# cyberlife-coder/velesdb

Measured on AMD Instinct MI355X. Metric: qps_at_recall10_1Mx768_k10, higher is better.
Workload: dtype f32; 1 GPU; 1000000x768 f32 cosine, k=10, exact distance sweep + fused GPU top-k (BASELINE configs[1]); 1024 queries/step, 1024 queries per corpus pass (sweep_topk_gemm_bf16_pp<dot, WIDE> over normalised bf16 images of rows and queries (cosine; ping-po; rows=1000000, dim=768, k=10, parallelism=replicas x1 (query stream split, no collective)

## Files before the change

velesdb_amd/csrc/g16_protocol.inc:

```
#ifndef VDB_PP_STAMP_AT
#define VDB_PP_STAMP_AT(SLOT) do { } while (0)
#define VDB_G16_OWN_STAMP_STUB 1
#endif
#ifndef VDB_PP_STAMP_COUNT
#define VDB_PP_STAMP_COUNT(SLOT) do { } while (0)
#define VDB_PP_STAMP_ADD(SLOT, N) do { } while (0)
#endif
    VDB_PP_STAMP_AT(16);
    if (hm[0] | hm[1] | hm[2] | hm[3]) VDB_PP_STAMP_COUNT(19);
    VDB_PP_STAMP_ADD(22, __popcll(hm[0]) + __popcll(hm[1]) + __popcll(hm[2]) + __popcll(hm[3]));
    for (;;) {
      ++epoch;
      VDB_PP_STAMP_COUNT(23);
      bool pend = false;
      {
        const uint32_t ln1 = lane_now();
        uint32_t fill = qcnt;
        uint32_t hsz = 64u;
        bool stop = false;
#define VDB_G16_SCAN(T) \
        while (hm[T] && !stop) { \
          if (hsz == 1u && fill + 32u > (uint32_t)QCAP) {  \
            stop = true; \
            break; \
          } \
          const uint32_t hrank = __builtin_amdgcn_mbcnt_hi((uint32_t)(hm[T] >> 32), __builtin_amdgcn_mbcnt_lo((uint32_t)hm[T], 0u)); \
          const bool mine = (((hm[T] >> ln1) & 1ull) != 0) & (hrank < hsz); \
          const uint64_t msk = __ballot(mine); \
          uint32_t nf = fill; \
          const uint32_t hi0 = ((uint32_t)(wr * 128) + 4u * (ln1 >> 4)) | (((uint32_t)(wq * 64 + (T) * 16) + (ln1 & 15u)) << 8); \
_Pragma("unroll") \
          for (int g8 = 0; g8 < 4; g8++) { \
            if (!__ballot(mine & (((gmv[T] >> g8) & 1u) != 0u))) continue;  \
_Pragma("unroll") \
            for (int j8 = 0; j8 < 8; j8++) { \
              float x; \
              VDB_G16_ACC_ELEM(x, acc[(8 * g8 + j8) >> 2][T][(8 * g8 + j8) & 3]);  \
               \
              const float xt = METRIC == kJaccard ? __builtin_fmaf(-cpv[T], vns[wr * 128 + 4 * (int)(ln1 >> 4) + ((8 * g8 + j8) >> 2) * 16 + ((8 * g8 + j8) & 3)], x) : x; \
              const bool pass = mine & !(xt < thrv[T]); \
              const uint64_t pm = __ballot(pass); \
              if (pm) { \
                if (pass) { \
                  const uint32_t slot = min(nf + __builtin_amdgcn_mbcnt_hi((uint32_t)(pm >> 32), __builtin_amdgcn_mbcnt_lo((uint32_t)pm, 0u)), (uint32_t)QCAP); \
                  uint32_t hi = hi0; \
                  asm volatile("" : "+v"(hi));  \
                  wq_keys[slot] = ((uint64_t)(hi + (uint32_t)(((8 * g8 + j8) >> 2) * 16 + ((8 * g8 + j8) & 3))) << 32) | (uint64_t)__float_as_uint(x); \
                } \
                nf += (uint32_t)__popcll(pm); \
              } \
            } \
          } \
          if (nf > (uint32_t)QCAP) {  \
            const uint32_t lanes = (uint32_t)__popcll(msk), room = (uint32_t)QCAP - fill; \
            hsz = lanes > 1u ? max(1u, min(lanes - 1u, lanes * room / (2u * (nf - fill)))) : 1u; \
            if (lanes == 1u) {  \
              stop = true; \
              break; \
            } \
            continue; \
          } \
          fill = nf; \
          hm[T] &= ~msk; \
        }
#define VDB_G16_FINISH(HAVE, RAW, FITS) do { \
          const uint64_t raw_ = (RAW); \
          const uint32_t b = (uint32_t)(raw_ >> 40) & 255u; \
          const float x = __uint_as_float((uint32_t)raw_); \
          const uint32_t rl = (uint32_t)(raw_ >> 32) & 255u; \
          const uint32_t row = rt * BM + rl; \
          float score; \
          if (METRIC == kHamming) {   \
            score = 0.5f * (qn[b] - x); \
          } else if (METRIC == kJaccard) {   \
            const float uni = qn[b] + vns[rl] - x; \
            score = uni == 0.0f ? 1.0f : x / uni; \
          } else { \
            score = halfp ? finish_score_half<METRIC>(x, qn[b], METRIC == kCosine ? vns[rl] : 1.0f) \
                          : finish_score<METRIC>(x, qn[b], METRIC == kCosine ? vns[rl] : 1.0f); \
          } \
           \
          if constexpr (WIDE) score = canon_nan(score); \
          const uint64_t key = make_key<HIB>(score, row); \
          bool take = (HAVE) & (row < a.n_rows) & (key < tauk[b]); \
          if (take && a.alive) take = a.alive[row] != 0;   \
          const uint64_t mt = __ballot(take); \
          FITS = qcnt + (uint32_t)__popcll(mt) <= (uint32_t)QCAP; \
          if (FITS) { \
            if (take) { \
              const uint32_t slot = qcnt + __builtin_amdgcn_mbcnt_hi((uint32_t)(mt >> 32), __builtin_amdgcn_mbcnt_lo((uint32_t)mt, 0u)); \
              wq_keys[slot] = key; \
              wq_qs[slot] = (uint8_t)b; \
            } \
            qcnt += (uint32_t)__popcll(mt); \
          } \
        } while (0)
#ifndef VDB_G16_NO_DUMP
        if ((uint32_t)__popcll(hm[0]) + (uint32_t)__popcll(hm[1]) + (uint32_t)__popcll(hm[2]) + (uint32_t)__popcll(hm[3]) <= (uint32_t)kG16DumpMaxLanes) {
          bool dump_ok = true;
          if (hm[0] | hm[1] | hm[2] | hm[3]) VDB_PP_STAMP_COUNT(21);
          float* dump = reinterpret_cast<float*>(wq_keys + 8);
#define VDB_G16_DUMP(T) \
          while (hm[T] && dump_ok) { \
            if (qcnt > 8u) { \
              dump_ok = false; \
              break; \
            } \
            VDB_PP_STAMP_COUNT(24);  \
            const uint32_t h0 = (uint32_t)__builtin_ctzll(hm[T]); \
            const uint64_t rest = hm[T] & (hm[T] - 1ull); \
            const uint32_t h1 = rest ? (uint32_t)__builtin_ctzll(rest) : 64u; \
            if (ln1 == h0 || ln1 == h1) { \
              f32x4* d = reinterpret_cast<f32x4*>(dump) + (ln1 == h1 ? 8 : 0); \
_Pragma("unroll") \
              for (int rf = 0; rf < 8; rf++) d[rf] = acc[rf][T]; \
            } \
            __builtin_amdgcn_fence(__ATOMIC_RELEASE, "wavefront"); \
            __builtin_amdgcn_wave_barrier(); \
            __builtin_amdgcn_fence(__ATOMIC_ACQUIRE, "wavefront"); \
            const uint32_t hs = ln1 < 32u ? h0 : h1;   \
            const uint32_t e = ln1 & 31u; \
            const float xd = dump[ln1]; \
            const uint32_t hi = ((((uint32_t)(wq * 64 + (T) * 16) + (hs & 15u)) << 8) | ((uint32_t)(wr * 128) + 4u * (hs >> 4) + (e >> 2) * 16u + (e & 3u))); \
            bool fits; \
            VDB_G16_FINISH(hs < 64u, ((uint64_t)hi << 32) | (uint64_t)__float_as_uint(xd), fits); \
            __builtin_amdgcn_wave_barrier();   \
            if (!fits) { \
              dump_ok = false; \
              break; \
            } \
            hm[T] = rest & (rest - 1ull); \
          }
          VDB_G16_DUMP(0)
          VDB_G16_DUMP(1)
          VDB_G16_DUMP(2)
          VDB_G16_DUMP(3)
#undef VDB_G16_DUMP
          fill = qcnt;
          VDB_PP_STAMP_AT(20);
        }
#endif
        if (gm_lazy && (hm[0] | hm[1] | hm[2] | hm[3])) {
#define VDB_G16_MASKS(T) do { if (METRIC == kJaccard) VDB_G16_GROUP_MASKS_J(T); else VDB_G16_GROUP_MASKS(T); } while (0)
          if (hm[0]) VDB_G16_MASKS(0);
          if (hm[1]) VDB_G16_MASKS(1);
          if (hm[2]) VDB_G16_MASKS(2);
          if (hm[3]) VDB_G16_MASKS(3);
#undef VDB_G16_MASKS
          gm_lazy = false;
        }
        for (;;) {
          VDB_G16_SCAN(0)
          VDB_G16_SCAN(1)
          VDB_G16_SCAN(2)
          VDB_G16_SCAN(3)
          VDB_PP_STAMP_AT(17);
          if (fill > qcnt) {
            const bool have = ln1 < fill - qcnt;
            const uint64_t raw = have ? wq_keys[qcnt + ln1] : 0ull;
            bool fits;
            VDB_G16_FINISH(have, raw, fits);
            (void)fits;
            fill = qcnt;
            VDB_PP_STAMP_AT(18);
          }
          if (!stop) break;
          if (qcnt + 32u > (uint32_t)QCAP) {
            pend = true;
            break;
          }
          stop = false;
        }
#undef VDB_G16_SCAN
#undef VDB_G16_FINISH
      }
      VDB_PP_STAMP_AT(12);
      if (pend || (last && qcnt)) flags[0] = epoch;
      __syncthreads();
      VDB_PP_STAMP_AT(13);
      if constexpr (!WIDE) {
      if (flags[1] == epoch) {
        compact();
        __syncthreads();
        VDB_PP_STAMP_AT(14);
      }
      }
      bool want = false;
      if constexpr (WIDE) {
        const uint32_t ln3 = lane_now();
        if (ln3 < qcnt) {
          const uint64_t key = wq_keys[ln3];
          const uint32_t qg = q0 + (uint32_t)wq_qs[ln3];
          const uint32_t idx = atomicAdd(&a.wide_cnt[qg], 1u);
          if (idx < a.wide_cap) a.wide_keys[(size_t)qg * a.wide_cap + idx] = key;
        }
        qcnt = 0;
      } else {
        const uint32_t ln3 = lane_now();
        const uint64_t key = ln3 < qcnt ? wq_keys[ln3] : kKeyInvalid;
        const uint32_t b = ln3 < qcnt ? wq_qs[ln3] : 0u;
        bool full = false;
        if (key != kKeyInvalid && key < tauk[b]) {
          const uint32_t idx = atomicAdd(&cnts[b], 1u);
          if (idx < (uint32_t)CAP) {
            cand[(size_t)b * CAP + idx] = key;
            want = idx >= k;
          } else {
            full = true;
            want = true;
          }
        }
        const uint64_t mf = __ballot(full);
        qcnt = (uint32_t)__popcll(mf);
        if (full) {
          const uint32_t slot = __builtin_amdgcn_mbcnt_hi((uint32_t)(mf >> 32), __builtin_amdgcn_mbcnt_lo((uint32_t)mf, 0u));
          wq_keys[slot] = key;
          wq_qs[slot] = (uint8_t)b;
        }
      }
      if (__ballot(want)) flags[1] = epoch + 1;
      VDB_PP_STAMP_AT(15);
      bool again = flags[0] >= epoch;
      if (last) {
        if (qcnt) flags[2] = epoch;
        __syncthreads();
        again |= flags[2] == epoch;
      }
      if (!again) break;
    }
#ifdef VDB_G16_OWN_STAMP_STUB
#undef VDB_PP_STAMP_AT
#undef VDB_G16_OWN_STAMP_STUB
#endif
```

velesdb_amd/csrc/g16_writeout.inc:

```
  if constexpr (!WIDE) {
  __syncthreads();
  compact();
  __syncthreads();
  const uint32_t lane_o = lane_now();
  for (uint32_t b = wib; b < nq_t; b += WAVES) {
    const uint32_t c = min(cnts[b], k);
    uint64_t* out = a.part_keys + ((size_t)(q0 + b) * a.list_stride + a.list_off + g) * k;
    for (uint32_t e = lane_o; e < k; e += 64) out[e] = e < c ? cand[(size_t)b * CAP + e] : kKeyInvalid;
    if (a.blk_tau && lane_o == 0) a.blk_tau[(size_t)(q0 + b) * a.list_stride + a.list_off + g] = tauk[b];
  }
  }
```

velesdb_amd/csrc/sweep_gemm_bf16.hip:

```cpp
#include <algorithm>

#include "vdb_probe_env.hpp"
#include "vdb_device.hpp"
#include "vdb_kernels.hpp"

namespace vdb {

typedef float f32x4 __attribute__((ext_vector_type(4)));
typedef __bf16 bf16x8 __attribute__((ext_vector_type(8)));
typedef __attribute__((address_space(3))) void* lds_ptr_t;
typedef __attribute__((address_space(3))) uint32_t lds_u32_t;

constexpr int kG16BM = 256, kG16BN = 256, kG16Waves = 8;
constexpr int kG16Cap = 12;
constexpr int kG16Queue = 39;
#ifndef VDB_G16_DUMP_MAX_LANES
#define VDB_G16_DUMP_MAX_LANES 6
#endif
constexpr int kG16DumpMaxLanes = VDB_G16_DUMP_MAX_LANES;
static_assert(kG16Queue == 39, "g16_protocol.inc keeps two hot lanes' 64 accumulators in queue entries 8 .. 39");
static_assert(kG16Queue <= 64 && kG16Queue >= 32, "the finish pass takes one queue entry per lane; one hot lane's 32 elements fit");
constexpr size_t kOffCand = 131072, kOffTauk = kOffCand + (size_t)kG16BN * kG16Cap * 8, kOffCnts = kOffTauk + kG16BN * 8,
                 kOffQn = kOffCnts + kG16BN * 4, kOffVns = kOffQn + kG16BN * 4, kOffFlags = kOffVns + kG16BM * 4,
                 kOffQueue = kOffFlags + 16,
                 kQueueBytes = 368,
                
                 kG16Lds = kOffQueue + kG16Waves * kQueueBytes;
static_assert(kG16Lds <= 160 * 1024, "LDS budget");
static_assert((size_t)(kG16Queue + 1) * 8 + kG16Queue + 4 <= 364 + 4 && (size_t)(kG16Queue + 1) * 8 + kG16Queue <= 364, "queue layout");

struct Bf16GemmArgs {
  const uint16_t* rows;
  const float* norms;
  const uint8_t* alive;
  const uint16_t* queries;
  const uint64_t* tau0;
  uint64_t* part_keys;
  uint64_t row_stride, q_stride;
  uint32_t n_rows, dim, nq, k;
  uint32_t KT, G, nqt, qper;
  uint32_t row_tile0;
  uint32_t list_stride, list_off;
  const float* qnorms;
  uint64_t* blk_tau;
  const float* qnorms_half;
  unsigned long long* dbg;
  uint64_t* wide_keys;
  uint32_t* wide_cnt;
  uint32_t wide_cap;
};

__device__ __forceinline__ uint32_t lane_now() {
  uint32_t l;
  asm volatile("v_mbcnt_lo_u32_b32 %0, -1, 0\n\tv_mbcnt_hi_u32_b32 %0, -1, %0" : "=v"(l));
  return l;
}

__device__ __forceinline__ void mfma_bf16_inplace(f32x4& c, const f32x4& a, const f32x4& b) {
  asm volatile("v_mfma_f32_16x16x32_bf16 %0, %1, %2, %0" : "+v"(c) : "v"(a), "v"(b));
}
__device__ __forceinline__ void mfma_bf16_first(f32x4& c, const f32x4& a, const f32x4& b) {
  asm volatile("v_mfma_f32_16x16x32_bf16 %0, %1, %2, 0" : "=&v"(c) : "v"(a), "v"(b));
}
__device__ __forceinline__ void mfma_drain() { asm volatile("s_nop 15\n\ts_nop 15" ::: "memory"); }

typedef int i32x4 __attribute__((ext_vector_type(4)));
__device__ __forceinline__ void glds_b128(const i32x4& rsrc, uint32_t voff, uint32_t soff, uint32_t lds_addr) {
  asm volatile("s_mov_b32 m0, %3\n\ts_nop 3\n\tbuffer_load_dwordx4 %0, %1, %2 offen lds"
               :
               : "v"(voff), "s"(rsrc), "s"(soff), "s"(lds_addr)
               : "m0");
}
__device__ __forceinline__ i32x4 make_rsrc(const void* base, uint32_t num_records = 0x7FFFFFFFu) {
  const uint64_t b = reinterpret_cast<uint64_t>(base);
  return i32x4{(int)(uint32_t)b, (int)((uint32_t)(b >> 32) & 0xFFFFu), (int)num_records, 0x00020000};
}
__device__ __forceinline__ i32x4 make_rsrc_uniform(const void* base, uint32_t num_records = 0x7FFFFFFFu) {
  const uint64_t b = reinterpret_cast<uint64_t>(base);
  const uint32_t lo = (uint32_t)__builtin_amdgcn_readfirstlane((int)(uint32_t)b);
  const uint32_t hi = (uint32_t)__builtin_amdgcn_readfirstlane((int)(uint32_t)(b >> 32));
  return i32x4{(int)lo, (int)(hi & 0xFFFFu), __builtin_amdgcn_readfirstlane((int)num_records), 0x00020000};
}
__device__ __forceinline__ uint32_t a_tile_records(uint32_t n_rows, uint32_t rt, uint32_t kt, uint64_t row_stride) {
  const uint64_t left = (uint64_t)(n_rows - rt * (uint32_t)kG16BM) * row_stride * 2u - (uint64_t)kt * 128u;
  return (uint32_t)(left < 0x7FFFFFFFull ? left : 0x7FFFFFFFull);
}
__device__ __forceinline__ uint32_t norm_records(uint32_t n_rows, uint32_t rt) {
  return min(n_rows - rt * (uint32_t)kG16BM, (uint32_t)kG16BM) * 4u;
}
__device__ __forceinline__ void wait_glds() { asm volatile("s_waitcnt vmcnt(0)" ::: "memory"); }

template <int METRIC, bool SPLIT>
__global__ __launch_bounds__(512, 2) void sweep_topk_gemm_bf16_glds(Bf16GemmArgs a) {
  constexpr bool HIB = true;
  constexpr bool WIDE = false;
  constexpr int BM = kG16BM, BN = kG16BN, WAVES = kG16Waves, CAP = kG16Cap, QCAP = kG16Queue;
  extern __shared__ __attribute__((aligned(16))) unsigned char smem[];
  uint64_t* cand = reinterpret_cast<uint64_t*>(smem + kOffCand);
  uint64_t* tauk = reinterpret_cast<uint64_t*>(smem + kOffTauk);
  uint32_t* cnts = reinterpret_cast<uint32_t*>(smem + kOffCnts);
  float* qn = reinterpret_cast<float*>(smem + kOffQn);
  float* vns = reinterpret_cast<float*>(smem + kOffVns);
  volatile lds_u32_t* flags = (volatile lds_u32_t*)(lds_ptr_t)(smem + kOffFlags);

  const int tid = (int)threadIdx.x;
  const int lane = tid & 63;
  const int wib = __builtin_amdgcn_readfirstlane(tid >> 6);
  const int wr = wib >> 2, wq = wib & 3;
  uint64_t* wq_keys = reinterpret_cast<uint64_t*>(smem + kOffQueue + (size_t)wib * kQueueBytes);
  uint8_t* wq_qs = reinterpret_cast<uint8_t*>(wq_keys + QCAP + 1);

  const uint32_t bid = blockIdx.x;
  const uint32_t xcd = bid & 7u, slot_id = bid >> 3;
  const uint32_t qt = slot_id % a.nqt;
  const uint32_t g = (slot_id / a.nqt) * 8u + xcd;
  const uint32_t q0 = qt * a.qper;
  const uint32_t nq_t = min(a.qper, a.nq - q0);
  const uint32_t k = a.k;
  const uint16_t* queries = a.queries + (size_t)q0 * a.q_stride;

  if (tid < BN) {
    cnts[tid] = 0;
    tauk[tid] = ((uint32_t)tid < nq_t && a.tau0) ? a.tau0[q0 + tid] : kKeyInvalid;
    qn[tid] = 0.0f;
  }
  if (tid < 4) flags[tid] = 0u;
  __syncthreads();
  if (a.qnorms) {
    if ((uint32_t)tid < nq_t) qn[tid] = a.qnorms[q0 + tid];
  } else if (a.qnorms_half) {
    if ((uint32_t)tid < nq_t) qn[tid] = a.qnorms_half[q0 + tid];
  } else {
    for (uint32_t b = wib; b < nq_t; b += WAVES) {
      const uint16_t* qp = queries + (size_t)b * a.q_stride;
      float nacc = 0.0f;
      for (uint32_t c = lane; c * 4 < a.dim; c += 64)
#pragma unroll
        for (int e = 0; e < 4; e++) {
          const uint32_t i = c * 4 + e;
          if (i < a.dim) {
            const float x = __uint_as_float((uint32_t)qp[i] << 16);
            nacc = __builtin_fmaf(x, x, nacc);
          }
        }
      const float n = sqrtf(butterfly_all(nacc));
      if (lane == 0) qn[b] = n;
    }
  }
  __syncthreads();
  const uint32_t ntiles = (a.n_rows + BM - 1) / BM;
  const uint32_t rt_first = a.row_tile0 + g;
  const uint32_t my_tiles = rt_first < ntiles ? (ntiles - rt_first + a.G - 1) / a.G : 0;
  const uint32_t total = my_tiles * a.KT;

  const uint32_t soff_a = 64u * (uint32_t)a.row_stride * 2u, soff_b = 64u * (uint32_t)a.q_stride * 2u;
  const unsigned char* rows_b = reinterpret_cast<const unsigned char*>(a.rows);
  const unsigned char* queries_b = reinterpret_cast<const unsigned char*>(queries);
  uint32_t ld_rt = rt_first, ld_kt = 0;
  const uint32_t lds0 = (uint32_t)(size_t)(lds_ptr_t)smem;
#define VDB_G16_REQ(BUF) \
    const uint32_t ln_ = lane_now(); \
    const uint32_t st_row = (uint32_t)wib * 8u + (ln_ >> 3); \
    const uint32_t st_slot = (ln_ & 7u) ^ ((st_row >> 1) & 7u); \
    const uint32_t voff_a = st_row * (uint32_t)a.row_stride * 2u + st_slot * 16u; \
    const uint32_t voff_b = st_row * (uint32_t)a.q_stride * 2u + st_slot * 16u; \
    const i32x4 ra = make_rsrc(rows_b + ((size_t)ld_rt * BM * a.row_stride + (size_t)ld_kt * 64) * 2, a_tile_records(a.n_rows, ld_rt, ld_kt, a.row_stride)); \
    const i32x4 rb = make_rsrc(queries_b + (size_t)ld_kt * 128); \
    const uint32_t la = lds0 + (uint32_t)(BUF) * 65536u + (uint32_t)wib * 1024u;
#define VDB_G16_GLDS(J) do { \
    if ((J) < 4) glds_b128(ra, voff_a, (uint32_t)(J) * soff_a, la + (uint32_t)(J) * 8192u); \
    else glds_b128(rb, voff_b, (uint32_t)((J) - 4) * soff_b, la + 32768u + (uint32_t)((J) - 4) * 8192u); \
  } while (0)
#define VDB_G16_ADVANCE() do { \
    if (it + 2 < total && ++ld_kt == a.KT) { \
      ld_kt = 0; \
      ld_rt += a.G; \
    } \
  } while (0)

  f32x4 acc[8][4];

#include "g16_compact.inc"
  uint32_t qcnt = 0;
  uint32_t epoch = 0;

#define VDB_G16_STEP(KT_NOW, FIRST) do { \
    const int buf = (int)(it & 1u); \
    VDB_G16_REQ(buf ^ 1) \
    if ((KT_NOW) == 0 && wib == 0)  \
      glds_b128(make_rsrc(reinterpret_cast<const unsigned char*>(a.norms) + (size_t)rt * BM * 4, norm_records(a.n_rows, rt)), ln_ * 16u, 0u, lds0 + (uint32_t)kOffVns); \
    const int sw_i = (int)((ln_ & 15u) >> 1) & 7; \
    const int rd_off = (int)(ln_ & 15u) * 128 + (((int)(ln_ >> 4) ^ sw_i) & 3) * 16; \
    const int rd_x = (sw_i & 4) << 4; \
    const int a_rd0 = wr * 128 * 128 + rd_off; \
    const int b_rd0 = 32768 + wq * 64 * 128 + rd_off; \
    const unsigned char* tb = smem + (size_t)buf * 65536; \
    if (!SPLIT) { \
_Pragma("unroll") \
      for (int m = 0; m < 2; m++) { \
        f32x4 av[8], bv[4]; \
_Pragma("unroll") \
        for (int t = 0; t < 4; t++) bv[t] = *reinterpret_cast<const f32x4*>(tb + b_rd0 + ((m * 64) ^ rd_x) + t * 2048); \
_Pragma("unroll") \
        for (int rf = 0; rf < 8; rf++) av[rf] = *reinterpret_cast<const f32x4*>(tb + a_rd0 + ((m * 64) ^ rd_x) + rf * 2048); \
_Pragma("unroll") \
        for (int rf = 0; rf < 8; rf++) { \
_Pragma("unroll") \
          for (int t = 0; t < 4; t++) { \
            if ((FIRST) && m == 0) mfma_bf16_first(acc[rf][t], av[rf], bv[t]); \
            else mfma_bf16_inplace(acc[rf][t], av[rf], bv[t]); \
          } \
          if (m == 0) VDB_G16_GLDS(rf); \
        } \
      } \
    } else {  \
      f32x4 bh[4], bl[4]; \
_Pragma("unroll") \
      for (int t = 0; t < 4; t++) { \
        bh[t] = *reinterpret_cast<const f32x4*>(tb + b_rd0 + (0 ^ rd_x) + t * 2048); \
        bl[t] = *reinterpret_cast<const f32x4*>(tb + b_rd0 + (64 ^ rd_x) + t * 2048); \
      } \
_Pragma("unroll") \
      for (int rp = 0; rp < 4; rp++) { \
        f32x4 ah[2], al[2]; \
_Pragma("unroll") \
        for (int i = 0; i < 2; i++) { \
          ah[i] = *reinterpret_cast<const f32x4*>(tb + a_rd0 + (0 ^ rd_x) + (rp * 2 + i) * 2048); \
          al[i] = *reinterpret_cast<const f32x4*>(tb + a_rd0 + (64 ^ rd_x) + (rp * 2 + i) * 2048); \
        } \
_Pragma("unroll") \
        for (int i = 0; i < 2; i++) \
_Pragma("unroll") \
          for (int t = 0; t < 4; t++) { \
            if (FIRST) mfma_bf16_first(acc[rp * 2 + i][t], ah[i], bh[t]); \
            else mfma_bf16_inplace(acc[rp * 2 + i][t], ah[i], bh[t]); \
          } \
        VDB_G16_GLDS(rp * 2); \
_Pragma("unroll") \
        for (int i = 0; i < 2; i++) \
_Pragma("unroll") \
          for (int t = 0; t < 4; t++) mfma_bf16_inplace(acc[rp * 2 + i][t], ah[i], bl[t]); \
        VDB_G16_GLDS(rp * 2 + 1); \
_Pragma("unroll") \
        for (int i = 0; i < 2; i++) \
_Pragma("unroll") \
          for (int t = 0; t < 4; t++) mfma_bf16_inplace(acc[rp * 2 + i][t], al[i], bh[t]); \
      } \
    } \
    VDB_G16_ADVANCE(); \
    it++; \
    wait_glds();  \
  } while (0)

  uint32_t it = 0;
  if (total) {
    VDB_G16_REQ(0)
#pragma unroll
    for (int j = 0; j < 8; j++) VDB_G16_GLDS(j);
    if (total > 1 && ++ld_kt == a.KT) {
      ld_kt = 0;
      ld_rt += a.G;
    }
    wait_glds();
  }
  __syncthreads();
  for (uint32_t rt = rt_first; rt < ntiles; rt += a.G) {
    VDB_G16_STEP(0, true);
    __syncthreads();
    for (uint32_t kt = 1; kt + 1 < a.KT; kt++) {
      VDB_G16_STEP(kt, false);
      __syncthreads();
    }
    VDB_G16_STEP(a.KT - 1, false);
    const bool more = it < total;
#define VDB_G16_ACC_F(V) (V)
#include "g16_quicktest.inc"
    if constexpr (METRIC == kHamming || METRIC == kJaccard) {
#include "g16_quicktest_bits.inc"
    } else {
#include "g16_quicktest_dense.inc"
    }
#define VDB_G16_ACC_ELEM(X, A) asm volatile("v_mov_b32 %0, %1" : "=v"(X) : "v"(A))
#define VDB_G16_NO_DUMP 1
#include "g16_protocol.inc"
#undef VDB_G16_NO_DUMP
#undef VDB_G16_ACC_ELEM
#undef VDB_G16_ACC_F
  }
#undef VDB_G16_STEP
#undef VDB_G16_ADVANCE
#undef VDB_G16_GLDS
#undef VDB_G16_REQ
#include "g16_writeout.inc"
}

template <bool FP4>
__device__ __forceinline__ void mfma_accv(f32x4& c, const f32x4& a, const f32x4& b) {
  if (FP4)
    asm volatile("v_mfma_scale_f32_16x16x128_f8f6f4 %0, %1, %2, %0, %3, %3 op_sel_hi:[0,0,0] cbsz:4 blgp:4" : "+v"(c) : "v"(a), "v"(b), "v"(0x7F7F7F7Fu));
  else
    asm volatile("v_mfma_f32_16x16x32_bf16 %0, %1, %2, %0" : "+v"(c) : "v"(a), "v"(b));
}
template <bool FP4>
__device__ __forceinline__ void mfma_accv_first(f32x4& c, const f32x4& a, const f32x4& b) {
  if (FP4)
    asm volatile("v_mfma_scale_f32_16x16x128_f8f6f4 %0, %1, %2, 0, %3, %3 op_sel_hi:[0,0,0] cbsz:4 blgp:4" : "=&v"(c) : "v"(a), "v"(b), "v"(0x7F7F7F7Fu));
  else
    asm volatile("v_mfma_f32_16x16x32_bf16 %0, %1, %2, 0" : "=&v"(c) : "v"(a), "v"(b));
}
template <int OFF>
__device__ __forceinline__ void lds_frag_read(f32x4& dst, uint32_t addr) {
  asm volatile("ds_read_b128 %0, %1 offset:%2" : "=v"(dst) : "v"(addr), "n"(OFF));
}
__device__ __forceinline__ void pp_barrier_reads_done() { asm volatile("s_waitcnt lgkmcnt(0)\n\ts_barrier" ::: "memory"); }
__device__ __forceinline__ void pp_barrier() { asm volatile("s_barrier" ::: "memory"); }
__device__ __forceinline__ void pp_wait_dma6() { asm volatile("s_waitcnt vmcnt(6)" ::: "memory"); }

template <int METRIC, bool FP4 = false, bool WIDE = false>
__global__ __launch_bounds__(512, 2) void sweep_topk_gemm_bf16_pp(Bf16GemmArgs a) {
  static_assert(FP4 == (METRIC == kHamming || METRIC == kJaccard), "the four-bit instance serves the bit metrics, the bf16 instance Cosine / DotProduct");
  constexpr bool HIB = METRIC != kHamming;
  constexpr int BM = kG16BM, BN = kG16BN, WAVES = kG16Waves, CAP = kG16Cap, QCAP = kG16Queue;
  extern __shared__ __attribute__((aligned(16))) unsigned char smem[];
  uint64_t* cand = reinterpret_cast<uint64_t*>(smem + kOffCand);
  uint64_t* tauk = reinterpret_cast<uint64_t*>(smem + kOffTauk);
  uint32_t* cnts = reinterpret_cast<uint32_t*>(smem + kOffCnts);
  float* qn = reinterpret_cast<float*>(smem + kOffQn);
  float* vns = reinterpret_cast<float*>(smem + kOffVns);
  volatile lds_u32_t* flags = (volatile lds_u32_t*)(lds_ptr_t)(smem + kOffFlags);

  const int tid = (int)threadIdx.x;
  const int lane = tid & 63;
  const int wib = __builtin_amdgcn_readfirstlane(tid >> 6);
  const int wr = wib >> 2, wq = wib & 3;
  uint64_t* wq_keys = reinterpret_cast<uint64_t*>(smem + kOffQueue + (size_t)wib * kQueueBytes);
  uint8_t* wq_qs = reinterpret_cast<uint8_t*>(wq_keys + QCAP + 1);

  const uint32_t bid = blockIdx.x;
  const uint32_t xcd = bid & 7u, slot_id = bid >> 3;
  const uint32_t qt = slot_id % a.nqt;
  const uint32_t g = (slot_id / a.nqt) * 8u + xcd;
  const uint32_t q0 = qt * a.qper;
  const uint32_t nq_t = min(a.qper, a.nq - q0);
  const uint32_t k = a.k;
  const uint16_t* queries = a.queries + (size_t)q0 * a.q_stride;

  if (tid < BN) {
    cnts[tid] = 0;
    tauk[tid] = ((uint32_t)tid < nq_t && a.tau0) ? a.tau0[q0 + tid] : kKeyInvalid;
    qn[tid] = 0.0f;
  }
  if (tid < 4) flags[tid] = 0u;
  __syncthreads();
  if (a.qnorms) {
    if ((uint32_t)tid < nq_t) qn[tid] = a.qnorms[q0 + tid];
  } else if (a.qnorms_half) {
    if ((uint32_t)tid < nq_t) qn[tid] = a.qnorms_half[q0 + tid];
  } else {
    for (uint32_t b = wib; b < nq_t; b += WAVES) {
      const uint16_t* qp = queries + (size_t)b * a.q_stride;
      float nacc = 0.0f;
      for (uint32_t c = lane; c * 4 < a.dim; c += 64)
#pragma unroll
        for (int e = 0; e < 4; e++) {
          const uint32_t i = c * 4 + e;
          if (i < a.dim) {
            const float x = __uint_as_float((uint32_t)qp[i] << 16);
            nacc = __builtin_fmaf(x, x, nacc);
          }
        }
      const float n = sqrtf(butterfly_all(nacc));
      if (lane == 0) qn[b] = n;
    }
  }
  __syncthreads();
  const uint32_t ntiles = (a.n_rows + BM - 1) / BM;
  const uint32_t rt_first = a.row_tile0 + g;
  const uint32_t my_tiles = rt_first < ntiles ? (ntiles - rt_first + a.G - 1) / a.G : 0;
  const uint32_t total = my_tiles * a.KT;

  uint32_t voff_a, voff_b;
  int a_rd0, b_rd0, rd_x;
#define VDB_PP_LANE() do { \
    const uint32_t ln_ = lane_now(); \
    const uint32_t st_row_ = (uint32_t)wib * 8u + (ln_ >> 3); \
    const uint32_t st_slot_ = (ln_ & 7u) ^ ((st_row_ >> 1) & 7u); \
    voff_a = st_row_ * (uint32_t)a.row_stride * 2u + st_slot_ * 16u; \
    voff_b = st_row_ * (uint32_t)a.q_stride * 2u + st_slot_ * 16u; \
    const int sw_i_ = (int)((ln_ & 15u) >> 1) & 7; \
    const int rd_off_ = (int)(ln_ & 15u) * 128 + (((int)(ln_ >> 4) ^ sw_i_) & 3) * 16; \
    rd_x = (sw_i_ & 4) << 4; \
    a_rd0 = wr * 128 * 128 + rd_off_; \
    b_rd0 = 32768 + wq * 64 * 128 + rd_off_; \
  } while (0)
  VDB_PP_LANE();
  const uint32_t soff_a = 64u * (uint32_t)a.row_stride * 2u, soff_b = 64u * (uint32_t)a.q_stride * 2u;
  const unsigned char* rows_b = reinterpret_cast<const unsigned char*>(a.rows);
  const unsigned char* queries_b = reinterpret_cast<const unsigned char*>(queries);
  const uint32_t lds0 = (uint32_t)(size_t)(lds_ptr_t)smem;
  const uint32_t lds_w = lds0 + (uint32_t)wib * 1024u;
#define VDB_PP_REQ_A(HALF, RT, KT_, BUF) do { \
    const i32x4 ra_ = make_rsrc_uniform(rows_b + ((size_t)(RT) * BM * a.row_stride + (size_t)(KT_) * 64) * 2, a_tile_records(a.n_rows, (RT), (KT_), a.row_stride)); \
    glds_b128(ra_, voff_a, (uint32_t)(2 * (HALF)) * soff_a, lds_w + (uint32_t)(BUF) * 65536u + (uint32_t)(2 * (HALF)) * 8192u); \
    glds_b128(ra_, voff_a, (uint32_t)(2 * (HALF) + 1) * soff_a, lds_w + (uint32_t)(BUF) * 65536u + (uint32_t)(2 * (HALF) + 1) * 8192u); \
  } while (0)
#define VDB_PP_REQ_B(HALF, KT_, BUF) do { \
    const i32x4 rb_ = make_rsrc_uniform(queries_b + (size_t)(KT_) * 128); \
    glds_b128(rb_, voff_b, (uint32_t)(2 * (HALF)) * soff_b, lds_w + (uint32_t)(BUF) * 65536u + 32768u + (uint32_t)(2 * (HALF)) * 8192u); \
    glds_b128(rb_, voff_b, (uint32_t)(2 * (HALF) + 1) * soff_b, lds_w + (uint32_t)(BUF) * 65536u + 32768u + (uint32_t)(2 * (HALF) + 1) * 8192u); \
  } while (0)

#define VDB_PP_READ_A(DST, RF0, BUF) do { \
    const uint32_t ad0_ = lds0 + (uint32_t)(BUF) * 65536u + (uint32_t)(a_rd0 + rd_x), ad1_ = lds0 + (uint32_t)(BUF) * 65536u + (uint32_t)(a_rd0 + (64 ^ rd_x)); \
    lds_frag_read<((RF0) + 0) * 2048>(DST[0][0], ad0_); lds_frag_read<((RF0) + 0) * 2048>(DST[0][1], ad1_); \
    lds_frag_read<((RF0) + 1) * 2048>(DST[1][0], ad0_); lds_frag_read<((RF0) + 1) * 2048>(DST[1][1], ad1_); \
    lds_frag_read<((RF0) + 2) * 2048>(DST[2][0], ad0_); lds_frag_read<((RF0) + 2) * 2048>(DST[2][1], ad1_); \
    lds_frag_read<((RF0) + 3) * 2048>(DST[3][0], ad0_); lds_frag_read<((RF0) + 3) * 2048>(DST[3][1], ad1_); \
  } while (0)
#define VDB_PP_READ_B(BUF) do { \
    const uint32_t bd0_ = lds0 + (uint32_t)(BUF) * 65536u + (uint32_t)(b_rd0 + rd_x), bd1_ = lds0 + (uint32_t)(BUF) * 65536u + (uint32_t)(b_rd0 + (64 ^ rd_x)); \
    lds_frag_read<0 * 2048>(bv[0][0], bd0_); lds_frag_read<0 * 2048>(bv[0][1], bd1_); \
    lds_frag_read<1 * 2048>(bv[1][0], bd0_); lds_frag_read<1 * 2048>(bv[1][1], bd1_); \
    lds_frag_read<2 * 2048>(bv[2][0], bd0_); lds_frag_read<2 * 2048>(bv[2][1], bd1_); \
    lds_frag_read<3 * 2048>(bv[3][0], bd0_); lds_frag_read<3 * 2048>(bv[3][1], bd1_); \
  } while (0)
#define VDB_PP_MFMA(AV, RF0, T0, FIRST) do { \
_Pragma("unroll") \
    for (int m_ = 0; m_ < 2; m_++) \
_Pragma("unroll") \
      for (int rf_ = 0; rf_ < 4; rf_++) \
_Pragma("unroll") \
        for (int t_ = 0; t_ < 2; t_++) { \
          if ((FIRST) && m_ == 0) mfma_accv_first<FP4>(acc[(RF0) + rf_][(T0) + t_], AV[rf_][m_], bv[(T0) + t_][m_]); \
          else mfma_accv<FP4>(acc[(RF0) + rf_][(T0) + t_], AV[rf_][m_], bv[(T0) + t_][m_]); \
        } \
  } while (0)

  f32x4 acc[8][4];
  f32x4 bv[4][2], a0v[4][2], a1v[4][2];

#include "g16_compact.inc"

  uint32_t qcnt = 0;
  uint32_t epoch = 0;

  uint32_t rt1 = rt_first, kt1 = 0, rt2 = rt_first, kt2 = 0, n2 = 0;
#define VDB_PP_NEXT2() do { \
    rt1 = rt2; \
    kt1 = kt2; \
    if (n2 + 1 < total) { \
      n2++; \
      if (++kt2 == a.KT) { \
        kt2 = 0; \
        rt2 += a.G; \
      } \
    } \
  } while (0)
  uint32_t c = 0;
  if (total) {
    VDB_PP_REQ_A(0, rt_first, 0, 0);
    VDB_PP_REQ_A(1, rt_first, 0, 0);
    VDB_PP_REQ_B(0, 0, 0);
    VDB_PP_REQ_B(1, 0, 0);
    VDB_PP_NEXT2();
    VDB_PP_REQ_B(0, kt2, 1);
    VDB_PP_REQ_A(0, rt2, kt2, 1);
    VDB_PP_REQ_A(1, rt2, kt2, 1);
    VDB_PP_NEXT2();
    pp_wait_dma6();
  }
  pp_barrier();
  if (total) VDB_PP_READ_A(a0v, 0, 0);
  if (wr == 1) pp_barrier();
#ifndef VDB_PP_STAMP
#define VDB_PP_STAMP 0
#endif
#ifndef VDB_PP_STAMP_METRIC
#define VDB_PP_STAMP_METRIC kCosine
#endif
#if VDB_PP_STAMP
  const bool st_on = a.dbg != nullptr && blockIdx.x == 8u && (wib == 0 || wib == 4) && METRIC == VDB_PP_STAMP_METRIC;
  uint32_t st_acc[28] = {0, 0, 0, 0, 0, 0, 0, 0, 0, 0, 0, 0, 0, 0, 0, 0, 0, 0, 0, 0, 0, 0, 0, 0, 0, 0, 0, 0};
  uint32_t st_last = 0;
#define VDB_PP_STAMP_AT(SLOT) do { \
    if (st_on) { \
      uint64_t t_; \
      asm volatile("s_memtime %0\n\ts_waitcnt lgkmcnt(0)" : "=s"(t_)::"memory"); \
      st_acc[SLOT] += (uint32_t)t_ - st_last; \
      st_last = (uint32_t)t_; \
    } \
  } while (0)
#define VDB_PP_STAMP_ISSUE(SLOT) do { if (VDB_PP_STAMP >= 2) VDB_PP_STAMP_AT(SLOT); } while (0)
#define VDB_PP_STAMP_COUNT(SLOT) do { if (st_on) st_acc[SLOT] += 1u; } while (0)
#define VDB_PP_STAMP_ADD(SLOT, N) do { if (st_on) st_acc[SLOT] += (uint32_t)(N); } while (0)
#else
#define VDB_PP_STAMP_AT(SLOT) do { } while (0)
#define VDB_PP_STAMP_ISSUE(SLOT) do { } while (0)
#endif
#define VDB_PP_LPART(READS, REQS) do { \
    READS; \
    REQS; \
  } while (0)
#define VDB_PP_KTILE(FIRST, LAST) do { \
    const uint32_t buf = c & 1u; \
     \
    VDB_PP_LPART(VDB_PP_READ_B(buf), VDB_PP_REQ_B(1, kt1, buf ^ 1u)); \
    if ((FIRST) && wib == 0)  \
      glds_b128(make_rsrc_uniform(reinterpret_cast<const unsigned char*>(a.norms) + (size_t)rt * BM * 4, norm_records(a.n_rows, rt)), lane_now() * 16u, 0u, lds0 + (uint32_t)kOffVns); \
    VDB_PP_STAMP_ISSUE(3); \
    pp_barrier_reads_done(); \
    VDB_PP_STAMP_AT(0); \
    VDB_PP_MFMA(a0v, 0, 0, FIRST); \
    VDB_PP_STAMP_AT(1); \
    pp_barrier(); \
    VDB_PP_STAMP_AT(2); \
     \
    VDB_PP_LPART(VDB_PP_READ_A(a1v, 4, buf), VDB_PP_REQ_B(0, kt2, buf)); \
    VDB_PP_STAMP_ISSUE(3); \
    pp_barrier_reads_done(); \
    VDB_PP_STAMP_AT(0); \
    VDB_PP_MFMA(a0v, 0, 2, FIRST); \
    VDB_PP_STAMP_AT(1); \
    pp_barrier(); \
    VDB_PP_STAMP_AT(2); \
     \
    VDB_PP_REQ_A(0, rt2, kt2, buf); \
    VDB_PP_STAMP_ISSUE(7); \
    pp_wait_dma6(); \
    pp_barrier_reads_done(); \
    VDB_PP_STAMP_AT(4); \
    VDB_PP_MFMA(a1v, 4, 2, FIRST); \
    VDB_PP_STAMP_AT(5); \
    pp_barrier(); \
    VDB_PP_STAMP_AT(6); \
     \
     \
    VDB_PP_LPART(if (!(LAST)) VDB_PP_READ_A(a0v, 0, buf ^ 1u), VDB_PP_REQ_A(1, rt2, kt2, buf)); \
    VDB_PP_STAMP_ISSUE(7); \
    pp_wait_dma6(); \
    pp_barrier_reads_done(); \
    VDB_PP_STAMP_AT(4); \
    VDB_PP_MFMA(a1v, 4, 0, FIRST); \
    VDB_PP_STAMP_AT(5); \
    pp_barrier(); \
    VDB_PP_STAMP_AT(6); \
    VDB_PP_NEXT2(); \
    c++; \
  } while (0)

#if VDB_PP_STAMP
  if (st_on) {
    uint64_t t_;
    asm volatile("s_memtime %0\n\ts_waitcnt lgkmcnt(0)" : "=s"(t_)::"memory");
    st_last = (uint32_t)t_;
  }
#endif
  for (uint32_t rt = rt_first; rt < ntiles; rt += a.G) {
    VDB_PP_KTILE(true, false);
    for (uint32_t kt = 1; kt + 1 < a.KT; kt++) VDB_PP_KTILE(false, false);
    VDB_PP_KTILE(false, true);
    const bool more = c < total;
    if (wr == 0) pp_barrier();
    VDB_PP_STAMP_AT(11);
#define VDB_G16_ACC_F(V) (V)
#include "g16_quicktest.inc"
    if constexpr (METRIC == kHamming || METRIC == kJaccard) {
#include "g16_quicktest_bits.inc"
    } else {
#include "g16_quicktest_dense.inc"
    }
    VDB_PP_STAMP_AT(10);
#define VDB_G16_ACC_ELEM(X, A) asm volatile("v_mov_b32 %0, %1" : "=v"(X) : "v"(A))
#include "g16_protocol.inc"
#undef VDB_G16_ACC_ELEM
#undef VDB_G16_ACC_F
    VDB_PP_LANE();
    VDB_PP_READ_A(a0v, 0, c & 1u);
    if (more && wr == 1) pp_barrier();
    VDB_PP_STAMP_AT(8);
  }
#undef VDB_PP_KTILE
#undef VDB_PP_LANE
#undef VDB_PP_NEXT2
#undef VDB_PP_MFMA
#undef VDB_PP_READ_B
#undef VDB_PP_READ_A
#undef VDB_PP_REQ_B
#undef VDB_PP_REQ_A
  asm volatile("s_waitcnt vmcnt(0)" ::: "memory");
#if VDB_PP_STAMP
  if (st_on && lane_now() == 0) {
    st_acc[9] = c;
    unsigned long long* d = a.dbg + (size_t)(wib == 0 ? 0 : 1) * 28;
    for (int i = 0; i < 28; i++) d[i] = st_acc[i];
  }
#endif
#include "g16_writeout.inc"
}

__global__ __launch_bounds__(256) void query_norms_bf16_kernel(const uint16_t* q16, uint64_t q_stride, float* out, uint32_t nq, uint32_t dim) {
  const uint32_t lane = threadIdx.x & 63u, b = blockIdx.x * 4u + (threadIdx.x >> 6);
  if (b >= nq) return;
  const uint16_t* qp = q16 + (size_t)b * q_stride;
  float nacc = 0.0f;
  for (uint32_t c = lane; c * 4 < dim; c += 64)
#pragma unroll
    for (int e = 0; e < 4; e++) {
      const uint32_t i = c * 4 + e;
      if (i < dim) {
        const float x = __uint_as_float((uint32_t)qp[i] << 16);
        nacc = __builtin_fmaf(x, x, nacc);
      }
    }
  const float n = sqrtf(butterfly_all(nacc));
  if (lane == 0) out[b] = n;
}
void launch_query_norms_bf16(const uint16_t* q16, uint64_t q_stride, float* out, uint32_t nq, uint32_t dim, hipStream_t st) {
  hipLaunchKernelGGL(query_norms_bf16_kernel, dim3((nq + 3) / 4), dim3(256), 0, st, q16, q_stride, out, nq, dim);
}

template <bool HIB>
__global__ __launch_bounds__(256) void seed_tau_kernel(const uint64_t* ids, const float* scores, const uint32_t* n, uint64_t* tau0,
                                                       uint64_t* list, uint32_t list_stride, uint32_t nq, uint32_t k) {
  const uint32_t q = blockIdx.x * 256 + threadIdx.x;
  if (q >= nq) return;
  const uint32_t c = min(n[q], k);
  uint64_t t = kKeyInvalid;
  if (c >= k && k > 0) t = make_key<HIB>(scores[(size_t)q * k + k - 1], (uint32_t)ids[(size_t)q * k + k - 1]) + 1ull;
  tau0[q] = t;
  if (list)
    for (uint32_t e = 0; e < k; e++)
      list[(size_t)q * list_stride * k + e] = e < c ? make_key<HIB>(scores[(size_t)q * k + e], (uint32_t)ids[(size_t)q * k + e]) : kKeyInvalid;
}
void launch_seed_tau(const uint64_t* ids, const float* scores, const uint32_t* n, uint64_t* tau0, uint64_t* list,
                     uint32_t list_stride, uint32_t nq, uint32_t k, hipStream_t st, bool hib) {
  if (hib) hipLaunchKernelGGL(seed_tau_kernel<true>, dim3((nq + 255) / 256), dim3(256), 0, st, ids, scores, n, tau0, list, list_stride, nq, k);
  else hipLaunchKernelGGL(seed_tau_kernel<false>, dim3((nq + 255) / 256), dim3(256), 0, st, ids, scores, n, tau0, list, list_stride, nq, k);
}

#if VDB_PP_STAMP
static unsigned long long* g_pp_stamp_buf = nullptr;
}
extern "C" int32_t vdb_hip_debug_pp_stamps(unsigned long long* out ) {
  if (!vdb::g_pp_stamp_buf) return -1;
  if (hipDeviceSynchronize() != hipSuccess) return -2;
  return hipMemcpy(out, vdb::g_pp_stamp_buf, 448, hipMemcpyDeviceToHost) == hipSuccess ? 0 : -3;
}
namespace vdb {
#endif
static_assert(kG16BM == (int)kGemmTileRows && kG16BN == (int)kGemmTileQueries, "the schedule's tile is the kernel's");

static bool pingpong_enabled() {
  static const bool on = [] {
    const char* e = probe_env("VELESDB_BF16_PP");
    return !(e && e[0] == '0');
  }();
  return on;
}
template <int METRIC>
static hipError_t launch_g16_pp(const Bf16GemmArgs& a, int blocks, hipStream_t st) {
  static bool done = false;
  if (!done) {
    hipError_t e = hipFuncSetAttribute(reinterpret_cast<const void*>(&sweep_topk_gemm_bf16_pp<METRIC>),
                                       hipFuncAttributeMaxDynamicSharedMemorySize, 160 * 1024);
    if (e != hipSuccess) return e;
    done = true;
  }
  hipLaunchKernelGGL((sweep_topk_gemm_bf16_pp<METRIC>), dim3(blocks), dim3(512), kG16Lds, st, a);
  return hipGetLastError();
}

template <int METRIC>
static hipError_t launch_g16_wide(const Bf16GemmArgs& a, int blocks, hipStream_t st) {
  static bool done = false;
  if (!done) {
    hipError_t e = hipFuncSetAttribute(reinterpret_cast<const void*>(&sweep_topk_gemm_bf16_pp<METRIC, false, true>),
                                       hipFuncAttributeMaxDynamicSharedMemorySize, 160 * 1024);
    if (e != hipSuccess) return e;
    done = true;
  }
  hipLaunchKernelGGL((sweep_topk_gemm_bf16_pp<METRIC, false, true>), dim3(blocks), dim3(512), kG16Lds, st, a);
  return hipGetLastError();
}

template <int METRIC>
static hipError_t launch_g16_fp4(const Bf16GemmArgs& a, int blocks, hipStream_t st) {
  static bool done = false;
  if (!done) {
    hipError_t e = hipFuncSetAttribute(reinterpret_cast<const void*>(&sweep_topk_gemm_bf16_pp<METRIC, true>),
                                       hipFuncAttributeMaxDynamicSharedMemorySize, 160 * 1024);
    if (e != hipSuccess) return e;
    done = true;
  }
  hipLaunchKernelGGL((sweep_topk_gemm_bf16_pp<METRIC, true>), dim3(blocks), dim3(512), kG16Lds, st, a);
  return hipGetLastError();
}

template <int METRIC, bool SPLIT>
static hipError_t launch_g16(const Bf16GemmArgs& a, int blocks, hipStream_t st) {
  static bool done = false;
  if (!done) {
    hipError_t e = hipFuncSetAttribute(reinterpret_cast<const void*>(&sweep_topk_gemm_bf16_glds<METRIC, SPLIT>),
                                       hipFuncAttributeMaxDynamicSharedMemorySize, 160 * 1024);
    if (e != hipSuccess) return e;
    done = true;
  }
  hipLaunchKernelGGL((sweep_topk_gemm_bf16_glds<METRIC, SPLIT>), dim3(blocks), dim3(512), kG16Lds, st, a);
  return hipGetLastError();
}

hipError_t launch_sweep_gemm_bf16_wide(int metric, const Bf16GemmPlan& p, const uint16_t* rows16, uint64_t row_stride, const float* norms,
                                       const uint8_t* alive, const uint16_t* queries16, uint64_t q_stride, const uint64_t* tau0,
                                       uint64_t* wide_keys, uint32_t* wide_cnt, uint32_t wide_cap, uint32_t dim, uint32_t nq, hipStream_t st,
                                       const float* qnorms) {
  Bf16GemmArgs a{};
  a.rows = rows16;
  a.norms = norms;
  a.alive = alive;
  a.queries = queries16;
  a.tau0 = tau0;
  a.row_stride = row_stride;
  a.q_stride = q_stride;
  a.n_rows = p.row_hi;
  a.row_tile0 = p.row_lo / kG16BM;
  a.dim = dim;
  a.nq = nq;
  a.k = kGemmBf16MaxK;
  a.KT = dim / 64;
  a.G = p.G;
  a.nqt = p.nqt;
  a.qper = p.qper;
  a.qnorms = qnorms;
  a.wide_keys = wide_keys;
  a.wide_cnt = wide_cnt;
  a.wide_cap = wide_cap;
  return metric == kCosine ? launch_g16_wide<kCosine>(a, p.blocks, st) : launch_g16_wide<kDot>(a, p.blocks, st);
}

hipError_t launch_sweep_gemm_bf16_glds(int metric, const Bf16GemmPlan& p, const uint16_t* rows16, uint64_t row_stride,
                                       const float* norms, const uint8_t* alive, const uint16_t* queries16, uint64_t q_stride,
                                       const uint64_t* tau0, uint64_t* part_keys, uint32_t list_stride, uint32_t list_off,
                                       uint32_t dim, uint32_t nq, uint32_t k, hipStream_t st, bool split, const float* qnorms,
                                       uint64_t* blk_tau, const float* qnorms_half) {
  Bf16GemmArgs a{};
  a.rows = rows16;
  a.norms = norms;
  a.alive = alive;
  a.queries = queries16;
  a.tau0 = tau0;
  a.part_keys = part_keys;
  a.row_stride = row_stride;
  a.q_stride = q_stride;
  a.n_rows = p.row_hi;
  a.row_tile0 = p.row_lo / kG16BM;
  a.list_stride = list_stride;
  a.list_off = list_off;
  a.dim = dim;
  a.nq = nq;
  a.k = k;
  a.KT = split ? dim / 32 : dim / 64;
  a.G = p.G;
  a.nqt = p.nqt;
  a.qper = p.qper;
  a.qnorms = qnorms;
  a.blk_tau = blk_tau;
  a.qnorms_half = qnorms_half;
#if VDB_PP_STAMP
  {
    static unsigned long long* dbg = [] {
      void* p = nullptr;
      if (hipMalloc(&p, 512) == hipSuccess) (void)hipMemset(p, 0, 512);
      return static_cast<unsigned long long*>(p);
    }();
    g_pp_stamp_buf = dbg;
    a.dbg = dbg;
  }
#endif
  if (metric == kHamming) return launch_g16_fp4<kHamming>(a, p.blocks, st);
  if (metric == kJaccard) return launch_g16_fp4<kJaccard>(a, p.blocks, st);
  if (split)
    return metric == kCosine ? launch_g16<kCosine, true>(a, p.blocks, st) : launch_g16<kDot, true>(a, p.blocks, st);
  if (pingpong_enabled()) return metric == kCosine ? launch_g16_pp<kCosine>(a, p.blocks, st) : launch_g16_pp<kDot>(a, p.blocks, st);
  return metric == kCosine ? launch_g16<kCosine, false>(a, p.blocks, st) : launch_g16<kDot, false>(a, p.blocks, st);
}

}
```

Measured before the change: 719,100 queries/s.

## Stage WIDE candidates in per-block LDS slots and flush once at writeout

In the WIDE path, each lane that passes the threshold now reserves a slot in the per-query LDS candidate array through an LDS atomic. Only candidates that overflow the per-block cap go straight to the global wide list. The wave-level queue, ballot compaction and per-epoch global atomics are removed, and the protocol loop exits after one pass. At writeout the block reserves global space per query with one atomic and copies the staged keys out, which cuts global atomic traffic in exchange for LDS atomics and an extra block barrier. It also factors the debug stamp buffer allocation into a helper and wires it into the wide launcher.

New measurement: 741,900 queries/s (median of 6 runs). 1.03x the previous value.

```diff
diff --git a/velesdb_amd/csrc/g16_protocol.inc b/velesdb_amd/csrc/g16_protocol.inc
--- a/velesdb_amd/csrc/g16_protocol.inc
+++ b/velesdb_amd/csrc/g16_protocol.inc
@@ -84,6 +84,20 @@
           const uint64_t key = make_key<HIB>(score, row); \
           bool take = (HAVE) & (row < a.n_rows) & (key < tauk[b]); \
           if (take && a.alive) take = a.alive[row] != 0;   \
+          if constexpr (WIDE) { \
+             \
+            if (take) { \
+              const uint32_t si = atomicAdd(&cnts[b], 1u); \
+              if (si < (uint32_t)CAP) { \
+                cand[(size_t)b * CAP + si] = key; \
+              } else { \
+                const uint32_t qg = q0 + b; \
+                const uint32_t gi = atomicAdd(&a.wide_cnt[qg], 1u); \
+                if (gi < a.wide_cap) a.wide_keys[(size_t)qg * a.wide_cap + gi] = key; \
+              } \
+            } \
+            FITS = true; \
+          } else { \
           const uint64_t mt = __ballot(take); \
           FITS = qcnt + (uint32_t)__popcll(mt) <= (uint32_t)QCAP; \
           if (FITS) { \
@@ -93,6 +107,7 @@
               wq_qs[slot] = (uint8_t)b; \
             } \
             qcnt += (uint32_t)__popcll(mt); \
+          } \
           } \
         } while (0)
 #ifndef VDB_G16_NO_DUMP
@@ -175,6 +190,11 @@
 #undef VDB_G16_FINISH
       }
       VDB_PP_STAMP_AT(12);
+      if constexpr (WIDE) {
+        __syncthreads();
+        VDB_PP_STAMP_AT(13);
+        break;
+      }
       if (pend || (last && qcnt)) flags[0] = epoch;
       __syncthreads();
       VDB_PP_STAMP_AT(13);
@@ -186,16 +206,7 @@
       }
       }
       bool want = false;
-      if constexpr (WIDE) {
-        const uint32_t ln3 = lane_now();
-        if (ln3 < qcnt) {
-          const uint64_t key = wq_keys[ln3];
-          const uint32_t qg = q0 + (uint32_t)wq_qs[ln3];
-          const uint32_t idx = atomicAdd(&a.wide_cnt[qg], 1u);
-          if (idx < a.wide_cap) a.wide_keys[(size_t)qg * a.wide_cap + idx] = key;
-        }
-        qcnt = 0;
-      } else {
+      {
         const uint32_t ln3 = lane_now();
         const uint64_t key = ln3 < qcnt ? wq_keys[ln3] : kKeyInvalid;
         const uint32_t b = ln3 < qcnt ? wq_qs[ln3] : 0u;
diff --git a/velesdb_amd/csrc/g16_writeout.inc b/velesdb_amd/csrc/g16_writeout.inc
--- a/velesdb_amd/csrc/g16_writeout.inc
+++ b/velesdb_amd/csrc/g16_writeout.inc
@@ -1,3 +1,18 @@
+  if constexpr (WIDE) {
+  __syncthreads();
+  uint32_t* wbase = reinterpret_cast<uint32_t*>(qn);
+  const uint32_t t_o = (uint32_t)wib * 64u + lane_now();
+  if (t_o < nq_t) {
+    const uint32_t n = min(cnts[t_o], (uint32_t)CAP);
+    wbase[t_o] = n ? atomicAdd(&a.wide_cnt[q0 + t_o], n) : 0u;
+  }
+  __syncthreads();
+  for (uint32_t i = t_o; i < nq_t * (uint32_t)CAP; i += (uint32_t)WAVES * 64u) {
+    const uint32_t b = i / (uint32_t)CAP, e = i - b * (uint32_t)CAP;
+    const uint32_t pos = wbase[b] + e;
+    if (e < cnts[b] && pos < a.wide_cap) a.wide_keys[(size_t)(q0 + b) * a.wide_cap + pos] = cand[i];
+  }
+  }
   if constexpr (!WIDE) {
   __syncthreads();
   compact();
diff --git a/velesdb_amd/csrc/sweep_gemm_bf16.hip b/velesdb_amd/csrc/sweep_gemm_bf16.hip
--- a/velesdb_amd/csrc/sweep_gemm_bf16.hip
+++ b/velesdb_amd/csrc/sweep_gemm_bf16.hip
@@ -640,6 +640,15 @@
 
 #if VDB_PP_STAMP
 static unsigned long long* g_pp_stamp_buf = nullptr;
+static unsigned long long* pp_stamp_dbg() {
+  static unsigned long long* dbg = [] {
+    void* p = nullptr;
+    if (hipMalloc(&p, 512) == hipSuccess) (void)hipMemset(p, 0, 512);
+    return static_cast<unsigned long long*>(p);
+  }();
+  g_pp_stamp_buf = dbg;
+  return dbg;
+}
 }
 extern "C" int32_t vdb_hip_debug_pp_stamps(unsigned long long* out ) {
   if (!vdb::g_pp_stamp_buf) return -1;
@@ -734,6 +743,9 @@
   a.wide_keys = wide_keys;
   a.wide_cnt = wide_cnt;
   a.wide_cap = wide_cap;
+#if VDB_PP_STAMP
+  a.dbg = pp_stamp_dbg();
+#endif
   return metric == kCosine ? launch_g16_wide<kCosine>(a, p.blocks, st) : launch_g16_wide<kDot>(a, p.blocks, st);
 }
 
@@ -766,15 +778,7 @@
   a.blk_tau = blk_tau;
   a.qnorms_half = qnorms_half;
 #if VDB_PP_STAMP
-  {
-    static unsigned long long* dbg = [] {
-      void* p = nullptr;
-      if (hipMalloc(&p, 512) == hipSuccess) (void)hipMemset(p, 0, 512);
-      return static_cast<unsigned long long*>(p);
-    }();
-    g_pp_stamp_buf = dbg;
-    a.dbg = dbg;
-  }
+  a.dbg = pp_stamp_dbg();
 #endif
   if (metric == kHamming) return launch_g16_fp4<kHamming>(a, p.blocks, st);
   if (metric == kJaccard) return launch_g16_fp4<kJaccard>(a, p.blocks, st);
```
